# ZhendongS/Physics-Informed-Neural-Network-for-Explainable-Fault-Diagnosis-in-Fuel-Cells

Measured on AMD Instinct MI355X. Metric: pinn_train_samples_per_s, higher is better.
Workload: dtype f32 (split-operand matrix products on the 16-bit matrix cores, f32 accumulate, fp32-matmul accuracy: 2 fp16 parts / 3 MFMAs per product in forward, backward and weight gradients); 1 GPU; BASELINE configs[1]: 1000000 synthetic rows x 8 features per GPU, PINN [8,256,256,256,1] + variance head, step = train_dnn (fwd+NLL+bwd+wgrad+allreduce+Adam) + one iteration of each of the 5 physics stages; rows_per_gpu=1000000, global_rows=1000000, parallelism=dp1, precision=f32x6, backend=none (single process), world_size=1

## Files before the change

physics-informed-neural-network-for-explainable-fault-diagnosis-in-fuel-cells_amd/csrc/pinn_x6_core.h:

```cpp
#pragma once
#include <type_traits>
#include <utility>
#include "pinn_bf16_core.h"

namespace pinn {
namespace x6 {

template <int I>
using IC = std::integral_constant<int, I>;
template <typename F, int... I>
__device__ __forceinline__ void static_for_impl(F&& f, std::integer_sequence<int, I...>) {
  (f(IC<I>{}), ...);
}
template <int N, typename F>
__device__ __forceinline__ void static_for(F&& f) {
  static_for_impl(f, std::make_integer_sequence<int, N>{});
}

constexpr int kThreadsX = 512;
constexpr int kTileRowsX = 128;
constexpr int kCopyLds = 16384;
constexpr int kSlabBytes = 3 * kCopyLds;

struct Mat {
  unsigned off;
  int nrb_log;
  int kp_log = 0;
  int rows_log = -1;
};
constexpr int clog2(int v) { return v <= 1 ? 0 : 1 + clog2(v >> 1); }

__device__ __forceinline__ int swz(int row) { return (0x78 >> (2 * ((row >> 2) & 3))) & 3; }

typedef __attribute__((address_space(1))) const void* gptr_t;
typedef __attribute__((address_space(3))) void* lptr_t;

#ifdef PINN_ABL_PLAINSTORE
#define PINN_STASH_ST(p, v) (*(p) = (v))
#else
#define PINN_STASH_ST(p, v) __builtin_nontemporal_store((v), (p))
#endif
#ifdef PINN_ABL_NTRING
#define PINN_RING_AUX 2
#else
#define PINN_RING_AUX 0
#endif
#ifdef PINN_X6_STAMP
__device__ unsigned long long g_x6_stamps[8 * 8];
__device__ __forceinline__ unsigned long long stamp() {
  unsigned long long t;
  __builtin_amdgcn_sched_barrier(0);
  asm volatile("s_memtime %0\n\ts_waitcnt lgkmcnt(0)" : "=s"(t) :: "memory");
  __builtin_amdgcn_sched_barrier(0);
  return t;
}
#define PINN_STAMP(pipe, k) do { const unsigned long long t_ = stamp(); (pipe).seg[k] += t_ - (pipe).last; (pipe).last = t_; } while (0)
#else
#define PINN_STAMP(pipe, k) do { } while (0)
#endif

template <int NCOPY>
struct PipeT {
  static constexpr int kSlab = NCOPY * kCopyLds;
#ifdef PINN_X6_STAMP
  unsigned long long seg[8], last;
#endif
  __amdgpu_buffer_rsrc_t rsrc;
  unsigned copy_bytes;
  char* lds;
  int par, wave;
  int read_off;
  unsigned lane_row2, lane_kq8;

  __device__ __forceinline__ void init(const void* packed, unsigned copy_bytes_, int tid) {
    rsrc = __builtin_amdgcn_make_buffer_rsrc(const_cast<void*>(packed), 0, 0x7FFFFFFF, 0x00020000);
    copy_bytes = __builtin_amdgcn_readfirstlane(copy_bytes_);
    wave = __builtin_amdgcn_readfirstlane(tid >> 6);
    read_off = 0;
    const int lane = tid & 63;
    lane_row2 = (unsigned)(lane >> 2) << 1;
    lane_kq8 = (unsigned)(((lane & 3) ^ swz(lane >> 2)) << 4);
  }
  template <int KP_LOG, int WAVES = 8>
  __device__ __forceinline__ void piece(const Mat& m, int g, int j, int buf) {
    int p = wave + WAVES * j;
    const int n = NCOPY << m.nrb_log;
    p = p < n ? p : p - n;
    asm volatile("" : "+s"(p));
    const int rs = m.rows_log >= 0 ? m.rows_log : m.nrb_log + 4;
    const unsigned voff = (lane_row2 << 5) + lane_kq8;
    const int copy = p >> m.nrb_log, rb = p & ((1 << m.nrb_log) - 1);
    const unsigned soff = (unsigned)copy * copy_bytes + 2u * (m.off + (((unsigned)g << rs) << 5) + (unsigned)rb * 512u);
    char* dst = lds + buf * kSlab + copy * kCopyLds + rb * 1024;
#ifndef PINN_ABL_NOPIECE
    __builtin_amdgcn_raw_ptr_buffer_load_lds(rsrc, (lptr_t)dst, 16, voff, soff, 0, 0);
#endif
  }
  template <int KP_LOG>
  __device__ __forceinline__ unsigned wave_base(const Mat& m) const { return 2u * m.off + (unsigned)wave * 1024u; }
  template <int KP_LOG, int WAVES, int NRB_LOG, int J>
  __device__ __forceinline__ void piece_s(unsigned mbase, int g, int buf) {
    constexpr int q = WAVES * J, copy = q >> NRB_LOG, rb0 = q & ((1 << NRB_LOG) - 1);
    static_assert(WAVES <= (1 << NRB_LOG) && copy < NCOPY, "piece_s: shape not separable");
    mbase = __builtin_amdgcn_readfirstlane(mbase);
    asm volatile("" : "+s"(mbase));
    const unsigned voff = (lane_row2 << 5) + lane_kq8;
    const unsigned soff = mbase + (unsigned)copy * copy_bytes + ((unsigned)g << (NRB_LOG + 10)) + (unsigned)rb0 * 1024u;
    char* dst = lds + buf * kSlab + wave * 1024 + copy * kCopyLds + rb0 * 1024;
#ifndef PINN_ABL_NOPIECE
    __builtin_amdgcn_raw_ptr_buffer_load_lds(rsrc, (lptr_t)dst, 16, voff, soff, 0, 0);
#endif
  }
  template <int KP_LOG, int WAVES = 8>
  __device__ __forceinline__ void prime(const Mat& first) {
    par = 0;
#pragma unroll
    for (int j = 0; j < 16 * NCOPY / WAVES; ++j)
      if (WAVES * j < (NCOPY << first.nrb_log)) piece<KP_LOG, WAVES>(first, 0, j, 0);
// ... 298 lines not shown
          PINN_STASH_ST(sp + r * 16, v0[r]);
          PINN_STASH_ST(sp + (16 + r) * 16, v1[r]);
        }
      }
    }
  }
}

template <typename S, int P, int NG, int NTOUT, int KPM, int KPN, int NPM, int NPN, bool kHasOut, int WAVES = 8, int kStIn = 0, int kStOut = 0,
          int NRBM = -1, typename FI, typename FO>
__device__ __forceinline__ void layer_x6(f32x4 (&acc)[NTOUT], typename S::Pipe& pipe, const Mat& mine, const Mat& next, int lane, PrepT<S>& st,
                                         FI&& prep_in, FO&& prep_out, bool out_on = true) {
  constexpr int kSlots = NTOUT / 2, kPerDma = (16 * S::kCopies / WAVES + kSlots - 1) / kSlots;
  constexpr int kFirst = kHasOut ? 2 : 0, kAvail = NTOUT - kFirst;
  static_assert(kAvail >= 1, "no chunk left for the next layer's group 0");
  static_assert(NRBM < 0 || NPM == (S::kCopies << NRBM), "NRBM does not match the piece count");
#ifdef PINN_ABL_GENERIC_PIECE
  constexpr int kNrbm = -1;
#else
  constexpr int kNrbm = NRBM;
#endif
  const unsigned mine_base = kNrbm >= 0 ? pipe.template wave_base<KPM>(mine) : 0u;
  static_for<NG>([&](auto gc) {
    constexpr int g = decltype(gc)::value;
    auto dma = [&](auto slotc) {
      static_for<kPerDma>([&](auto qc) {
        constexpr int j = decltype(slotc)::value * kPerDma + decltype(qc)::value;
        if constexpr (g + 1 < NG) {
          if constexpr (WAVES * j < NPM) {
            if constexpr (kNrbm >= 0) pipe.template piece_s<KPM, WAVES, kNrbm, j>(mine_base, g + 1, pipe.par ^ 1);
            else pipe.template piece<KPM, WAVES>(mine, g + 1, j, pipe.par ^ 1);
          }
        } else {
          if constexpr (WAVES * j < NPN) pipe.template piece<KPN, WAVES>(next, 0, j, pipe.par ^ 1);
        }
      });
    };
    auto vchunk = [&](auto cc) {
      constexpr int c = decltype(cc)::value;
      static_for<7>([&](auto kc) {
        constexpr int k = decltype(kc)::value;
        if constexpr ((k < 6 && kFirst + k * kAvail / 6 == c) || (k == 6 && c == NTOUT - 1)) {
          if constexpr (g + 1 < NG) prep_in(IC<g + 1>{}, IC<k>{}, st.buf[(P + g + 1) & 1]);
          else if constexpr (kHasOut) prep_out(IC<k>{}, st.buf[(P + g + 1) & 1]);
        }
      });
    };
    slab_mfma<S, NTOUT>(acc, st.buf[(P + g) & 1], pipe.cur(), lane, vchunk, dma);
    PINN_STAMP(pipe, (NTOUT == 16 ? 0 : NTOUT == 8 ? 1 : 2));
    if constexpr (g + 1 < NG) pipe.template advance<kStIn>();
    else if constexpr (kHasOut && kStOut > 0) { if (out_on) pipe.template advance<kStOut>(); else pipe.template advance<0>(); }
    else pipe.template advance<0>();
    PINN_STAMP(pipe, 4 + (NTOUT == 16 ? 0 : NTOUT == 8 ? 1 : 2));
  });
}

template <typename S, int kThreads>
__device__ __forceinline__ void fill_small(float* small, float* w0t, const float* __restrict__ params, const ParamLayout& L) {
  const SmallLayout SL{L.H, L.nh};
  const int Hh = L.H, tid = threadIdx.x;
  constexpr int kMaxH = 256, kPer = (kMaxH + kThreads - 1) / kThreads;
  constexpr int kW0 = (8 * kMaxH + kThreads - 1) / kThreads, kMaxLayers = 8;
  float vb[kMaxLayers][kPer], vwp[kPer], vbv0[kPer], vbv1[kPer], vwv2[kPer], vw0[kW0], vbp = 0.f, vbv2 = 0.f;
#pragma unroll
  for (int l = 0; l < kMaxLayers; ++l)
#pragma unroll
    for (int k = 0; k < kPer; ++k) { const int i = tid + k * kThreads; vb[l][k] = (l < L.nh && i < Hh) ? params[L.b(l) + i] : 0.f; }
#pragma unroll
  for (int k = 0; k < kPer; ++k) {
    const int i = tid + k * kThreads;
    vwp[k] = i < Hh ? params[L.wp() + i] : 0.f;
    vbv0[k] = i < Hh / 2 ? params[L.bv0() + i] : 0.f;
    vbv1[k] = i < Hh / 4 ? params[L.bv1() + i] : 0.f;
    vwv2[k] = i < Hh / 4 ? params[L.wv2() + i] : 0.f;
  }
#pragma unroll
  for (int k = 0; k < kW0; ++k) { const int e = tid + k * kThreads; vw0[k] = e < Hh * 8 ? params[L.w0() + e] : 0.f; }
  if (tid == 0) { vbp = params[L.bp()]; vbv2 = params[L.bv2()]; }
#pragma unroll
  for (int l = 0; l < kMaxLayers; ++l)
#pragma unroll
    for (int k = 0; k < kPer; ++k) { const int i = tid + k * kThreads; if (l < L.nh && i < Hh) small[SL.b(l) + i] = l == 0 ? vb[l][k] : vb[l][k] * S::kAccScale; }
#pragma unroll
  for (int k = 0; k < kPer; ++k) {
    const int i = tid + k * kThreads;
    if (i < Hh) small[SL.wp() + i] = vwp[k];
    if (i < Hh / 2) small[SL.bv0() + i] = vbv0[k] * S::kAccScale;
    if (i < Hh / 4) { small[SL.bv1() + i] = vbv1[k] * S::kAccScale; small[SL.wv2() + i] = vwv2[k]; }
  }
#pragma unroll
  for (int k = 0; k < kW0; ++k) { const int e = tid + k * kThreads; if (e < Hh * 8) w0t[(e & 7) * kW0Stride + (e >> 3)] = vw0[k]; }
  if (tid == 0) { small[SL.bp()] = vbp; small[SL.bv2()] = vbv2; }
  __syncthreads();
}

__device__ __forceinline__ int lane_of(const RowCtx& c) { return c.lane; }

template <int H>
__device__ __forceinline__ Mat first_mat(const PackLayout& K) {
  return K.nh > 1 ? Mat{(unsigned)K.w(1), clog2(H / 16)} : Mat{(unsigned)K.wv0(), clog2(H / 32)};
}

__device__ __forceinline__ float* packed_ptr(float* base, long long t16, int F, int lane) {
  return base + t16 * F * 16 + (lane & 15) * 16 + (lane >> 4) * 4;
}

struct StashX {
  float* h; float* v1; float* v2;
  float* dh; float* dv1; float* dv2;
  long long t16_total, t16;
  __device__ __forceinline__ float* act(int layer, int H_, int lane) const {
    return tiled_ptr(h + (long long)layer * t16_total * H_ * 16, t16, H_, lane);
  }
  __device__ __forceinline__ float* dact(int layer, int H_, int lane) const {
    return tiled_ptr(dh + (long long)layer * t16_total * H_ * 16, t16, H_, lane);
  }
  __device__ __forceinline__ float* actp(int layer, int H_, int lane) const {
    return packed_ptr(h + (long long)layer * t16_total * H_ * 16, t16, H_, lane);
  }
  __device__ __forceinline__ float* dactp(int layer, int H_, int lane) const {
    return packed_ptr(dh + (long long)layer * t16_total * H_ * 16, t16, H_, lane);
  }
};

template <typename S, int H, bool kBits, bool TRAIN = false, int WAVES = 8, bool kPack = false>
__device__ __forceinline__ void forward_pass(const float* w0t, const float* smallp, const ParamLayout& L, typename S::Pipe& pipe,
                                             const DropDev& d, const RowCtx& c, const f32x4& xa, const f32x4& xb, float& u, float& z,
                                             const StashX* sx = nullptr) {
  static_assert(!kPack || (TRAIN && S::kCopies == 2), "the packed stash holds scheme X3's fragments");
  constexpr int NT = H / 16, NT2 = H / 32, NT4 = H / 64, NP = H / 32, NC = S::kCopies;
  constexpr int kSt = TRAIN ? (kPack ? 2 : 8) : 0;
  auto act_ptr = [&](int layer) -> float* { return kPack ? sx->actp(layer, H, lane_of(c)) : sx->act(layer, H, lane_of(c)); };
  auto v1_ptr = [&]() -> float* { return kPack ? packed_ptr(sx->v1, sx->t16, H / 2, lane_of(c)) : tiled_ptr(sx->v1, sx->t16, H / 2, lane_of(c)); };
  using Frag = typename S::Frag;
  const int lane = c.lane, kq = c.kq;
  const SmallLayout SL{L.H, L.nh};
  const PackLayout K{L.H, L.nh};
  constexpr int KPW = clog2(H), KPV1 = clog2((H / 2 + 63) & ~63);
  const Mat m_v0{(unsigned)K.wv0(), clog2(H / 32)}, m_v1{(unsigned)K.wv1(), clog2(H / 64)};
  const float* wp = smallp + SL.wp();
  const int ll = L.nh - 1;
  constexpr float kPre0 = kTanhPre, kPreS = kTanhPre / S::kAccScale;
  auto drop_of = [&](int layer) { LayerDrop ld = layer_drop(d, c.mode, layer); ld.scale *= S::kActScale; return ld; };
  float up = 0.0f;
  PrepT<S> st;
  f32x4 h[NT];
  layer_input_lds<NT>(h, w0t, smallp + SL.b(0), xa, xb, lane);
  {
    const LayerDrop ld0 = drop_of(0);
    float* sp = TRAIN ? act_ptr(0) : nullptr;
    static_for<7>([&](auto kc) { prep_micro<S, kBits, true, decltype(kc)::value, 0, kPack>(st, h[0], h[1], d, c, ld0, kPre0, 0, wp, up, ll == 0, st.buf[0], sp); });
  }
#pragma unroll 1
  for (int l = 1; l < L.nh; ++l) {
    f32x4 acc[NT];
    bias_blocks<NT>(acc, smallp + SL.b(l), kq);
    const LayerDrop ld_in = drop_of(l - 1), ld_out = drop_of(l);
    const float pre_in = l == 1 ? kPre0 : kPreS;
    const bool last = l == ll;
    const Mat mine{(unsigned)K.w(l), clog2(H / 16)}, next = last ? m_v0 : Mat{(unsigned)K.w(l + 1), clog2(H / 16)};
    float* sp_in = TRAIN ? act_ptr(l - 1) : nullptr;
    float* sp_out = TRAIN ? act_ptr(l) : nullptr;
    static_assert(NP % 2 == 0 && (NP / 2) % 2 == 0, "the forward layers keep the fragment buffer parity");
    layer_x6<S, 0, NP, NT, KPW, KPW, NC * H / 16, NC * H / 16, true, WAVES, kSt, kSt, clog2(H / 16)>(
        acc, pipe, mine, next, lane, st,
        [&](auto gc, auto kc, Frag& out) {
          constexpr int g = decltype(gc)::value;
          prep_micro<S, kBits, false, decltype(kc)::value, g, kPack>(st, h[2 * g], h[2 * g + 1], d, c, ld_in, pre_in, l - 1, wp, up, false, out,
                                                                    TRAIN ? sp_in + 32 * g * 16 : nullptr);
        },
        [&](auto kc, Frag& out) {
          prep_micro<S, kBits, true, decltype(kc)::value, 0, kPack>(st, acc[0], acc[1], d, c, ld_out, kPreS, l, wp, up, last, out, sp_out);
        });
#pragma unroll
    for (int t = 0; t < NT; ++t) h[t] = acc[t];
  }
  f32x4 v1[NT2];
  bias_blocks<NT2>(v1, smallp + SL.bv0(), kq);
  {
    const LayerDrop ld_in = drop_of(ll), ld_out = drop_of(L.nh);
    const float pre_in = ll == 0 ? kPre0 : kPreS;
    float* sp_in = TRAIN ? act_ptr(ll) : nullptr;
    float* sp_out = TRAIN ? v1_ptr() : nullptr;
    layer_x6<S, 0, NP, NT2, KPW, KPV1, NC * H / 32, NC * H / 64, true, WAVES, kSt, kSt, (WAVES <= H / 32 ? clog2(H / 32) : -1)>(
        v1, pipe, m_v0, m_v1, lane, st,
        [&](auto gc, auto kc, Frag& out) {
          constexpr int g = decltype(gc)::value;
          prep_micro<S, kBits, true, decltype(kc)::value, g, kPack>(st, h[2 * g], h[2 * g + 1], d, c, ld_in, pre_in, ll, wp + 32 * g, up, true, out,
                                                                   TRAIN ? sp_in + 32 * g * 16 : nullptr);
        },
        [&](auto kc, Frag& out) {
          prep_micro<S, kBits, false, decltype(kc)::value, 0, kPack>(st, v1[0], v1[1], d, c, ld_out, kPreS, L.nh, wp, up, false, out, sp_out);
        });
  }
  u = sum_kq(up) + smallp[SL.bp()];
  f32x4 v2[NT4];
  bias_blocks<NT4>(v2, smallp + SL.bv1(), kq);
  {
    const LayerDrop ld_in = drop_of(L.nh);
    float* sp_in = TRAIN ? v1_ptr() : nullptr;
    auto prep_in = [&](auto gc, auto kc, Frag& out) {
      constexpr int g = decltype(gc)::value;
      prep_micro<S, kBits, false, decltype(kc)::value, g, kPack>(st, v1[2 * g], v1[2 * g + 1], d, c, ld_in, kPreS, L.nh, wp, up, false, out,
                                                                TRAIN ? sp_in + 32 * g * 16 : nullptr);
    };
// ... 29 lines not shown
};

struct StashFrag {
  u32x4 hi, lo;
};
template <int B, int R>
__device__ __forceinline__ float unpack_act(const StashFrag& f) {
  const unsigned hw = f.hi[R], lw = f.lo[R];
  const f16x2 h = __builtin_bit_cast(f16x2, hw), l = __builtin_bit_cast(f16x2, lw);
  return (float)h[B] + (float)l[B];
}

__device__ __forceinline__ int grad_exponent(float mx, int e_if_zero) {
  int e = 0;
  (void)frexpf(mx, &e);
  return (mx > 0.0f && mx < __builtin_inff()) ? (e < -120 ? -120 : e) : e_if_zero;
}

template <typename S, int k>
__device__ __forceinline__ void bprep_micro(typename S::Frag& out, f32x4& d0, f32x4& d1, const StashRing& ring, int buf, float* dsp, float gscale,
                                            float inv_scale, float unnorm, float& mx, StashFrag& sf) {
  constexpr bool kPack = S::kCopies == 2;
  if constexpr (k == 1) {
    if constexpr (kPack) { sf.hi = ring.read_frag(buf, 0); sf.lo = ring.read_frag(buf, 1); }
  } else if constexpr (k >= 2 && k < 6) {
    constexpr int r = k - 2;
    const float h0 = kPack ? unpack_act<0, r>(sf) : ring.read(buf, 0, r), h1 = kPack ? unpack_act<1, r>(sf) : ring.read(buf, 1, r);
    const float a0 = h0 * inv_scale, a1 = h1 * inv_scale;
    const float g0 = d0[r] * (gscale * (1.0f - a0 * a0)), g1 = d1[r] * (gscale * (1.0f - a1 * a1));
    const float p0 = h0 != 0.0f ? g0 : 0.0f, p1 = h1 != 0.0f ? g1 : 0.0f;
    d0[r] = p0; d1[r] = p1;
    S::template split<r>(p0, p1, out);
  } else if constexpr (k == 6) {
    if constexpr (kPack) {
      PINN_STASH_ST(reinterpret_cast<u32x4*>(dsp), out.hi);
      PINN_STASH_ST(reinterpret_cast<u32x4*>(dsp + 256), out.lo);
#pragma unroll
      for (int r = 0; r < 4; ++r) mx = fmaxf(fmaxf(mx, fabsf(d0[r])), fabsf(d1[r]));
    } else {
#pragma unroll
      for (int r = 0; r < 4; ++r) {
        PINN_STASH_ST(dsp + r * 16, S::kActScale != 1.0f ? d0[r] * unnorm : d0[r]);
        PINN_STASH_ST(dsp + (16 + r) * 16, S::kActScale != 1.0f ? d1[r] * unnorm : d1[r]);
        if constexpr (S::kActScale != 1.0f) mx = fmaxf(fmaxf(mx, fabsf(d0[r])), fabsf(d1[r]));
      }
    }
  }
}

struct RowMeta {
  _Float16* rec;
  int E, c;
};
template <typename S, int H, int WAVES = 8>
__device__ __forceinline__ void backward_pass(const float* smallp, const ParamLayout& L, typename S::Pipe& pipe, const DropDev& d, int mode,
                                              const StashX& sx, const StashRing& ring, int lane, float du, float dz, float& amax,
                                              const RowMeta meta = RowMeta{nullptr, 4, 0}) {
  constexpr int NT = H / 16, NT2 = H / 32, NT4 = H / 64, NP = H / 32, NC = S::kCopies;
  constexpr int NG1 = (H / 4) / 32 > 0 ? (H / 4) / 32 : 1;
  constexpr int KPW = clog2(H), KPT0 = clog2((H / 2 + 63) & ~63), KPT1 = clog2((H / 4 + 63) & ~63);
  constexpr bool kPack = NC == 2;
  constexpr int kSt = kPack ? 2 : 8;
  using Frag = typename S::Frag;
  const int kq = lane >> 4;
  const SmallLayout SL{L.H, L.nh};
  const PackLayout K{L.H, L.nh};
  const int nh = L.nh;
  const int n_blocks = NP / 2 + (nh - 1) * NP;
  auto block_ptr = [&](int i) -> const float* {
    if (i < NP / 2) return sx.v1 + (sx.t16 * (H / 2) + 32 * i) * 16;
    const int j = i - NP / 2, layer = nh - 1 - j / NP, g = j % NP;
    return sx.h + ((long long)layer * sx.t16_total * H + sx.t16 * H + 32 * g) * 16;
  };
  auto fetch_block = [&](int i) {
    if (i < n_blocks) ring.fetch(block_ptr(i), i & 1);
  };
  fetch_block(0);

  float unnorm = 1.0f;
  float mx = 0.0f;
  if constexpr (S::kActScale != 1.0f) {
    const int e = grad_exponent(fmaxf(fabsf(du), fabsf(dz)), kPack ? meta.E : 4);
    const float norm = ldexpf(1.0f, 4 - e);
    unnorm = ldexpf(1.0f, e - 4);
    if constexpr (kPack) {
      if (meta.rec && lane < 16) reinterpret_cast<float*>(meta.rec)[32 + lane] = dz;
    }
    du *= norm; dz *= norm;
    if constexpr (kPack) {
      if (meta.rec && lane < 16) {
        const _Float16 dh16 = (_Float16)du;
        meta.rec[lane] = (_Float16)ldexpf(1.0f, e - meta.E + meta.c);
        meta.rec[16 + lane] = dh16;
        meta.rec[32 + lane] = (_Float16)(du - (float)dh16);
      }
    }
  }
  constexpr float kInvW = 1.0f / (S::kAccScale / S::kActScale);
  constexpr float kInvA = kPack ? 1.0f / S::kActScale : 1.0f;

  PrepT<S> st;
  StashFrag sf;
  constexpr int P1 = NG1 & 1;
  f32x4 v2[NT4];
  float* dsp2 = kPack ? packed_ptr(sx.dv2, sx.t16, H / 4, lane) : tiled_ptr(sx.dv2, sx.t16, H / 4, lane);
  {
    const float* vp = tiled_ptr(sx.v2, sx.t16, H / 4, lane);
#pragma unroll
    for (int t = 0; t < NT4; ++t) load_block(vp, t, v2[t]);
#pragma unroll
    for (int t = 0; t < NT4; ++t) {
      const f32x4 w = *reinterpret_cast<const f32x4*>(smallp + SL.wv2() + t * 16 + 4 * kq);
      f32x4 true_units;
#pragma unroll
      for (int r = 0; r < 4; ++r) {
        v2[t][r] = w[r] * dz * (1.0f - v2[t][r] * v2[t][r]);
        true_units[r] = v2[t][r] * unnorm;
        if constexpr (S::kActScale != 1.0f) mx = fmaxf(mx, fabsf(v2[t][r]));
      }
      if constexpr (!kPack) store_block(dsp2, t, true_units);
    }
    const f32x4 zero = {0.f, 0.f, 0.f, 0.f};
    const f32x4& second = NT4 >= 2 ? v2[NT4 >= 2 ? 1 : 0] : zero;
    static_for<4>([&](auto rc) { constexpr int r = decltype(rc)::value; S::template split<r>(v2[0][r], second[r], st.buf[0]); });
    if constexpr (kPack) {
      PINN_STASH_ST(reinterpret_cast<u32x4*>(dsp2), st.buf[0].hi);
      PINN_STASH_ST(reinterpret_cast<u32x4*>(dsp2 + 256), st.buf[0].lo);
    }
  }
  const Mat m_t1{(unsigned)K.wv1t(), clog2(H / 32)}, m_t0{(unsigned)K.wv0t(), clog2(H / 16)};
  const Mat m_again{m_t1.off, m_t1.nrb_log, KPT1};
  auto dv1_ptr = [&]() -> float* { return kPack ? packed_ptr(sx.dv1, sx.t16, H / 2, lane) : tiled_ptr(sx.dv1, sx.t16, H / 2, lane); };
  auto dact_ptr = [&](int layer) -> float* { return kPack ? sx.dactp(layer, H, lane) : sx.dact(layer, H, lane); };

  f32x4 dpv1[NT2];
  zero_blocks<NT2>(dpv1);
  {
    const LayerDrop ldv = layer_drop(d, mode, nh);
    const float gscale = ldv.scale * kInvW, inv_scale = kInvA / ldv.scale;
    float* dsp = dv1_ptr();
    layer_x6<S, 0, NG1, NT2, KPT1, KPT0, NC * H / 32, NC * H / 16, true, WAVES, (kPack ? 2 : 0), kSt, (WAVES <= H / 32 ? clog2(H / 32) : -1)>(
        dpv1, pipe, m_t1, m_t0, lane, st,
        [&](auto gc, auto kc, Frag& out) {
          constexpr int g = decltype(gc)::value, k = decltype(kc)::value;
          if constexpr (k >= 2 && k < 6 && 2 * g + 1 < NT4) S::template split<k - 2>(v2[2 * g][k - 2], v2[2 * g + 1][k - 2], out);
          if constexpr (kPack && k == 6 && 2 * g + 1 < NT4) {
            PINN_STASH_ST(reinterpret_cast<u32x4*>(dsp2 + 512 * g), out.hi);
            PINN_STASH_ST(reinterpret_cast<u32x4*>(dsp2 + 512 * g + 256), out.lo);
          }
        },
        [&](auto kc, Frag& out) {
          constexpr int k = decltype(kc)::value;
          if constexpr (k == 0) {
            asm volatile("s_waitcnt vmcnt(0)" ::: "memory");
            fetch_block(1);
          }
          bprep_micro<S, k>(out, dpv1[0], dpv1[1], ring, 0, dsp, gscale, inv_scale, unnorm, mx, sf);
        });
  }

  f32x4 dh[NT];
#pragma unroll
  for (int t = 0; t < NT; ++t) {
    const f32x4 w = *reinterpret_cast<const f32x4*>(smallp + SL.wp() + t * 16 + 4 * kq);
    dh[t] = w * (du * (S::kAccScale / S::kActScale));
  }
  {
    const LayerDrop ldv = layer_drop(d, mode, nh), ldh = layer_drop(d, mode, nh - 1);
    const float gscale = ldv.scale * kInvW, inv_scale = kInvA / ldv.scale, gscale_o = ldh.scale * kInvW, inv_scale_o = kInvA / ldh.scale;
    float* dsp = dv1_ptr();
    float* dsp_o = dact_ptr(nh - 1);
    const Mat next = nh > 1 ? Mat{(unsigned)K.wt(nh - 1), clog2(H / 16), KPW} : m_again;
    layer_x6<S, P1, NP / 2, NT, KPT0, -1, NC * H / 16, NC * H / 16, true, WAVES, kSt, kSt, clog2(H / 16)>(
        dh, pipe, m_t0, next, lane, st,
        [&](auto gc, auto kc, Frag& out) {
          constexpr int g = decltype(gc)::value, k = decltype(kc)::value;
          if constexpr (k == 0) fetch_block(g + 1);
          bprep_micro<S, k>(out, dpv1[2 * g], dpv1[2 * g + 1], ring, g & 1, dsp + 32 * g * 16, gscale, inv_scale, unnorm, mx, sf);
        },
        [&](auto kc, Frag& out) {
          constexpr int k = decltype(kc)::value;
          if (nh > 1) {
            if constexpr (k == 0) fetch_block(NP / 2 + 1);
            bprep_micro<S, k>(out, dh[0], dh[1], ring, (NP / 2) & 1, dsp_o, gscale_o, inv_scale_o, unnorm, mx, sf);
          }
        },
        nh > 1);
  }

#pragma unroll 1
  for (int l = nh - 1; l >= 1; --l) {
    f32x4 acc[NT];
    zero_blocks<NT>(acc);
    const LayerDrop ld_in = layer_drop(d, mode, l), ld_out = layer_drop(d, mode, l - 1);
    const float gscale = ld_in.scale * kInvW, inv_scale = kInvA / ld_in.scale, gscale_o = ld_out.scale * kInvW, inv_scale_o = kInvA / ld_out.scale;
    float* dsp = dact_ptr(l);
    float* dsp_o = dact_ptr(l - 1);
    const int base = NP / 2 + (nh - 1 - l) * NP;
    const Mat mine{(unsigned)K.wt(l), clog2(H / 16)}, next = l > 1 ? Mat{(unsigned)K.wt(l - 1), clog2(H / 16), KPW} : m_again;
    layer_x6<S, P1, NP, NT, KPW, -1, NC * H / 16, NC * H / 16, true, WAVES, kSt, kSt, clog2(H / 16)>(
        acc, pipe, mine, next, lane, st,
        [&](auto gc, auto kc, Frag& out) {
          constexpr int g = decltype(gc)::value, k = decltype(kc)::value;
          if constexpr (k == 0) fetch_block(base + g + 1);
          bprep_micro<S, k>(out, dh[2 * g], dh[2 * g + 1], ring, (base + g) & 1, dsp + 32 * g * 16, gscale, inv_scale, unnorm, mx, sf);
        },
        [&](auto kc, Frag& out) {
          constexpr int k = decltype(kc)::value;
          if (l > 1) {
            if constexpr (k == 0) fetch_block(base + NP + 1);
            bprep_micro<S, k>(out, acc[0], acc[1], ring, (base + NP) & 1, dsp_o, gscale_o, inv_scale_o, unnorm, mx, sf);
          }
        },
        l > 1);
#pragma unroll
    for (int t = 0; t < NT; ++t) dh[t] = acc[t];
  }

  {
    const LayerDrop ld0 = layer_drop(d, mode, 0);
    const float gscale = ld0.scale * kInvW * (kPack ? 1.0f : unnorm), inv_scale = kInvA / ld0.scale;
    auto one = [&](float h, float dv) -> float {
      const float a0 = h * inv_scale;
      const float g0 = dv * (gscale * (1.0f - a0 * a0));
      return h != 0.0f ? g0 : 0.0f;
    };
    if constexpr (kPack) {
      const float* hp = sx.actp(0, H, lane);
      float* dsp = sx.dactp(0, H, lane);
      StashFrag fr[NP];
// ... 40 lines not shown
```

physics-informed-neural-network-for-explainable-fault-diagnosis-in-fuel-cells_amd/csrc/pinn_x6_train.hip:

```cpp
#include <cstdlib>
#include "pinn_x6_core.h"

namespace pinn {
namespace x6 {

struct TrainArgsX {
  const float* params;
  const float* x;
  const float* y;
  long long n_rows, n_global;
  int H, nh;
  DropDev drop;
  TrainBuffers b;
};

template <int H, bool kBits, int WAVES, bool kPack>
__global__ __launch_bounds__(WAVES * 64, WAVES / 4) void train_fwd_x3_kernel(TrainArgsX a, const __bf16* packed) {
  using S = X3;
  constexpr int kThreadsX = WAVES * 64, kTileRowsX = WAVES * 16;
  constexpr int kSmallBytes = kMaxSmall * 4, kW0Bytes = 8 * kW0Stride * 4, kRedBytes = 8 * kLossTerms * 8;
  constexpr int kSlabAt = (kSmallBytes + kW0Bytes + kRedBytes + 1023) & ~1023;
  __shared__ __attribute__((aligned(1024))) char smem[kSlabAt + 2 * S::Pipe::kSlab];
  float* small = reinterpret_cast<float*>(smem);
  float* w0t = reinterpret_cast<float*>(smem + kSmallBytes);
  double (*red)[kLossTerms] = reinterpret_cast<double (*)[kLossTerms]>(smem + kSmallBytes + kW0Bytes);
  char* lds_w = smem + kSlabAt;
  ParamLayout L{a.H, a.nh};
  PackLayout K{a.H, a.nh};
  fill_small<S, kThreadsX>(small, w0t, a.params, L);
  S::Pipe pipe;
  pipe.lds = lds_w;
  pipe.init(packed + 3 * K.total(), (unsigned)(K.total() * 2), threadIdx.x);
  pipe.template prime<clog2(H), WAVES>(first_mat<H>(K));

  const int lane = threadIdx.x & 63, wave = pipe.wave, kq = lane >> 4;
  const float inv_n = (float)(1.0 / (double)a.n_global);
  LossSums sums;
  float gmax = 0.f;
  if (blockIdx.x == 0 && threadIdx.x == 0) *a.b.amax = 0u;

  const long long n_tiles = (a.n_rows + 127) / 128 * (128 / kTileRowsX);
  const unsigned pass0 = train_pass(a.drop);
  if (blockIdx.x == 0 && threadIdx.x == 0) a.b.amax[2] = pass0;
  for (long long tile = blockIdx.x; tile < n_tiles; tile += gridDim.x) {
    const long long t16 = tile * WAVES + wave;
    const long long lrow = t16 * 16 + (lane & 15);
    const bool valid = lrow < a.n_rows;
    const long long srow = valid ? lrow : a.n_rows - 1;
    const f32x4 xa = reinterpret_cast<const f32x4*>(a.x)[srow * 2];
    const f32x4 xb = reinterpret_cast<const f32x4*>(a.x)[srow * 2 + 1];
    const float yv = a.y[srow];
    const RowCtx c{lane, kq, a.drop.row_offset + lrow, srow, a.n_rows, pass0, a.drop.mode};
    const StashX sx{(float*)a.b.stash_h, (float*)a.b.stash_v1, (float*)a.b.stash_v2, (float*)a.b.dpre_h, (float*)a.b.dpre_v1, (float*)a.b.dpre_v2,
                    a.b.t16, t16};

    if constexpr (kPack) {
      Frag2 fx;
      static_for<4>([&](auto rc) {
        constexpr int r = decltype(rc)::value;
        const float v = kq == 0 ? xa[r] : (kq == 1 ? xb[r] : 0.0f);
        S::template split<r>(v * 0.0625f, 0.0f, fx);
      });
      float* xp = packed_ptr((float*)a.b.stash_x, t16, 32, lane);
      PINN_STASH_ST(reinterpret_cast<u32x4*>(xp), fx.hi);
      PINN_STASH_ST(reinterpret_cast<u32x4*>(xp + 256), fx.lo);
    }
    float u, z;
    forward_pass<S, H, kBits, true, WAVES, kPack>(w0t, small, L, pipe, a.drop, c, xa, xb, u, z, &sx);

    float du, dz;
    loss_row(u, z, yv, inv_n, valid, kq == 0, du, dz, sums);
    if (lane < 16) { a.b.du[t16 * 16 + lane] = du; a.b.dz[t16 * 16 + lane] = dz; }
    gmax = fmaxf(gmax, fmaxf(fabsf(du), fabsf(dz)));
  }
  if constexpr (kPack) wave_max_to(a.b.emax, gmax, lane == 0);

  store_loss_partials<WAVES>(sums, red, a.b.loss_part, lane, wave);
}

template <typename S, int H, int WAVES>
__global__ __launch_bounds__(WAVES * 64, WAVES / 4) void train_bwd_kernel(TrainArgsX a, const __bf16* packed) {
  constexpr int kThreadsX = WAVES * 64, kTileRowsX = WAVES * 16;
  constexpr int kSmallBytes = kMaxSmall * 4, kW0Bytes = 8 * kW0Stride * 4, kRingBytes = 8 * 2 * 2048;
  constexpr int kSlabAt = (kSmallBytes + kW0Bytes + kRingBytes + 1023) & ~1023;
  __shared__ __attribute__((aligned(1024))) char smem[kSlabAt + 2 * S::Pipe::kSlab];
  float* small = reinterpret_cast<float*>(smem);
  float* w0t = reinterpret_cast<float*>(smem + kSmallBytes);
  char* ring_lds = smem + kSmallBytes + kW0Bytes;
  char* lds_w = smem + kSlabAt;
  ParamLayout L{a.H, a.nh};
  PackLayout K{a.H, a.nh};
  fill_small<X6, kThreadsX>(small, w0t, a.params, L);
  typename S::Pipe pipe;
  pipe.lds = lds_w;
  pipe.init(packed + (S::kCopies == 2 ? 3 * K.total() : 0), (unsigned)(K.total() * 2), threadIdx.x);
  constexpr int KPT1 = clog2((H / 4 + 63) & ~63);
  pipe.template prime<KPT1, WAVES>(Mat{(unsigned)K.wv1t(), clog2(H / 32)});

  const int lane = threadIdx.x & 63, wave = pipe.wave;
  const StashRing ring{ring_lds + wave * 4096, lane};
  const long long n_tiles = (a.n_rows + 127) / 128 * (128 / kTileRowsX);
  float amax = 0.0f;
  int E = 4;
  if constexpr (S::kCopies == 2) E = grad_exponent(__builtin_bit_cast(float, __builtin_amdgcn_readfirstlane(*a.b.emax)), 4);
  for (long long tile = blockIdx.x; tile < n_tiles; tile += gridDim.x) {
    const long long t16 = tile * WAVES + wave;
    const StashX sx{(float*)a.b.stash_h, (float*)a.b.stash_v1, (float*)a.b.stash_v2, (float*)a.b.dpre_h, (float*)a.b.dpre_v1, (float*)a.b.dpre_v2,
                    a.b.t16, t16};
    const float du = a.b.du[t16 * 16 + (lane & 15)], dz = a.b.dz[t16 * 16 + (lane & 15)];
    const RowMeta meta{S::kCopies == 2 ? (_Float16*)a.b.rowmeta + t16 * 128 : nullptr, E, a.b.qboost};
    backward_pass<S, H, WAVES>(small, L, pipe, a.drop, a.drop.mode, sx, ring, lane, du, dz, amax, meta);
  }
  if constexpr (S::kActScale != 1.0f) wave_max_to(a.b.amax, amax, lane == 0);
}

#ifdef PINN_ABL_Q_NTSTORE
#define PINN_Q_ST(p, v) __builtin_nontemporal_store((v), (p))
#else
#define PINN_Q_ST(p, v) (*(p) = (v))
#endif
struct Xch {
  char* base;
  int off;
  __device__ __forceinline__ u32x4 read(int g, int part) const { return *reinterpret_cast<const u32x4*>(base + g * 2048 + part * 1024 + off); }
  __device__ __forceinline__ void write(int g, const Frag2& f) const {
    *reinterpret_cast<u32x4*>(base + g * 2048 + off) = f.hi;
    *reinterpret_cast<u32x4*>(base + g * 2048 + 1024 + off) = f.lo;
  }
};
__device__ __forceinline__ void lds_barrier() {
  asm volatile("s_waitcnt lgkmcnt(0)" ::: "memory");
  __builtin_amdgcn_s_barrier();
  asm volatile("" ::: "memory");
}
template <bool kDot>
__device__ __forceinline__ void prep_group(Frag2& out, const f32x4& v0, const f32x4& v1, const DropDev& d, const RowCtx& c, const LayerDrop ld,
                                           float pre, int layer, int fp, const float* wp32, float& up) {
  unsigned keep = 0u;
  if (c.mode == PINN_DROP_BITS) {
    const unsigned word = d.bits[((long long)c.pass * c.n_rows + c.lrow) * d.words + layer * d.nb + fp];
    const unsigned lo = (word >> (4 * c.kq)) & 0xFu, hi = (word >> (16 + 4 * c.kq)) & 0xFu;
    keep = ld.thr == 0 ? 0xFFu : (lo | (hi << 4));
  } else {
    PrepBase s;
    s.w0 = (unsigned)c.grow; s.w1 = (unsigned)((unsigned long long)c.grow >> 32);
    s.w2 = ((unsigned)layer << 16) | ((unsigned)fp << 2) | (unsigned)c.kq; s.w3 = d.stream + c.pass;
    philox_rounds5<0>(s, d.seed_lo, d.seed_hi);
    philox_rounds5<5>(s, d.seed_lo, d.seed_hi);
    static_for<4>([&](auto rc) {
      constexpr int r = decltype(rc)::value;
      keep |= (keep_draw<0, r>(s, ld.thr) ? 1u : 0u) << r;
      keep |= (keep_draw<1, r>(s, ld.thr) ? 1u : 0u) << (4 + r);
    });
  }
  const float m2s = -2.0f * ld.scale;
  static_for<4>([&](auto rc) {
    constexpr int r = decltype(rc)::value;
    float a0 = fmaf(m2s, __builtin_amdgcn_rcpf(__builtin_amdgcn_exp2f(v0[r] * pre) + 1.0f), ld.scale);
    float a1 = fmaf(m2s, __builtin_amdgcn_rcpf(__builtin_amdgcn_exp2f(v1[r] * pre) + 1.0f), ld.scale);
    a0 = a0 == 0.0f ? 0x1p-24f : a0;
    a1 = a1 == 0.0f ? 0x1p-24f : a1;
    const float hs0 = ((keep >> r) & 1u) ? a0 : 0.0f, hs1 = ((keep >> (4 + r)) & 1u) ? a1 : 0.0f;
    X3::split<r>(hs0, hs1, out);
    if constexpr (kDot) {
      const float h0 = hs0 * (1.0f / X3::kActScale), h1 = hs1 * (1.0f / X3::kActScale);
// ... 304 lines not shown
int train_chain_x6_partials(const pinn_net_t* net, long long n_rows) { return x6::plan_chain(net, n_rows).grid_fwd; }

int launch_train_chain_x6(const pinn_net_t* net, const float* d_params, const float* d_x, const float* d_y, long long n_rows,
                          long long n_global, const DropDev& drop, const TrainBuffers& b, unsigned which, void* stream) {
  using namespace x6;
  hipStream_t st = (hipStream_t)stream;
  const bool fast_bwd = net->precision == PINN_PREC_F32X6;
  const bool run_fwd = which & 1u, fwd_only = !(which & 2u);
  launch_pack_x6(net, d_params, st, fast_bwd && run_fwd ? b.emax : nullptr);
  TrainArgsX a{};
  a.params = d_params; a.x = d_x; a.y = d_y; a.n_rows = n_rows; a.n_global = n_global; a.H = net->hidden; a.nh = net->n_hidden;
  a.drop = drop; a.b = b;
  const ChainPlan c = plan_chain(net, n_rows);
  const bool small_n = c.small_n;
  const int grid = c.grid;
  const __bf16* packed = (const __bf16*)net->d_packed;
  const bool bits = drop.mode == PINN_DROP_BITS;
  if (c.quarters) {
    if (run_fwd) hipLaunchKernelGGL((train_fwd_small_kernel<256>), dim3(c.grid_fwd), dim3(kSmallThreads), 0, st, a, packed);
    if (!fwd_only) {
      if (!run_fwd) { hipError_t em = hipMemsetAsync(b.amax, 0, sizeof(unsigned), st); if (em != hipSuccess) return (int)em; }
      hipLaunchKernelGGL((train_bwd_kernel<X3, 256, 4>), dim3(grid), dim3(256), 0, st, a, packed);
    }
    hipError_t eq = hipGetLastError();
    return eq == hipSuccess ? PINN_OK : (int)eq;
  }
  if (fast_bwd && !fwd_only && !run_fwd) {
    hipError_t em = hipMemsetAsync(b.amax, 0, sizeof(unsigned), st);
    if (em != hipSuccess) return (int)em;
  }
#define PINN_LAUNCH_T(HH, BB)                                                                                                   \
  do {                                                                                                                          \
    if (small_n) {                                                                                                              \
      if (run_fwd && fast_bwd) hipLaunchKernelGGL((train_fwd_x3_kernel<HH, BB, 4, true>), dim3(grid), dim3(256), 0, st, a, packed);   \
      else if (run_fwd) hipLaunchKernelGGL((train_fwd_x3_kernel<HH, BB, 4, false>), dim3(grid), dim3(256), 0, st, a, packed);   \
      if (!fwd_only && fast_bwd) hipLaunchKernelGGL((train_bwd_kernel<X3, HH, 4>), dim3(grid), dim3(256), 0, st, a, packed);    \
      else if (!fwd_only) hipLaunchKernelGGL((train_bwd_kernel<X6, HH, 4>), dim3(grid), dim3(256), 0, st, a, packed);           \
    } else {                                                                                                                    \
      if (run_fwd && fast_bwd) hipLaunchKernelGGL((train_fwd_x3_kernel<HH, BB, 8, true>), dim3(grid), dim3(512), 0, st, a, packed);   \
      else if (run_fwd) hipLaunchKernelGGL((train_fwd_x3_kernel<HH, BB, 8, false>), dim3(grid), dim3(512), 0, st, a, packed);   \
      if (!fwd_only && fast_bwd) hipLaunchKernelGGL((train_bwd_kernel<X3, HH, 8>), dim3(grid), dim3(512), 0, st, a, packed);    \
      else if (!fwd_only) hipLaunchKernelGGL((train_bwd_kernel<X6, HH, 8>), dim3(grid), dim3(512), 0, st, a, packed);           \
    }                                                                                                                           \
  } while (0)
  if (net->hidden == 256) { if (bits) PINN_LAUNCH_T(256, true); else PINN_LAUNCH_T(256, false); }
  else { if (bits) PINN_LAUNCH_T(128, true); else PINN_LAUNCH_T(128, false); }
#undef PINN_LAUNCH_T
  hipError_t e = hipGetLastError();
  return e == hipSuccess ? PINN_OK : (int)e;
}

}

#ifdef PINN_Q_STAMP
extern "C" int pinn_q_debug_read(unsigned long long* host) {
  return (int)hipMemcpyFromSymbol(host, HIP_SYMBOL(pinn::x6::g_q_stamps), sizeof(unsigned long long) * 8 * 16);
}
#endif
```

Baseline: 227.6 million samples/s.

## Prefetch next tile's inputs into LDS across the tile seam in fwd and bwd kernels

In the forward kernel, each wave's x/y rows for the next tile are fetched into a double-buffered LDS stage with global_load_lds, issued after the first layer prep. In the backward kernel, the next tile's du/dz, v2 stash and first v1 ring block are fetched during the current tile. The first fetches are issued before fill_small and weight priming so they overlap. The aim is to hide global-load latency at tile boundaries, at the cost of extra LDS and a removed vmcnt wait that could create ordering hazards. Optional seam timing stamps are added behind a macro.

```diff
diff --git a/physics-informed-neural-network-for-explainable-fault-diagnosis-in-fuel-cells_amd/csrc/pinn_x6_core.h b/physics-informed-neural-network-for-explainable-fault-diagnosis-in-fuel-cells_amd/csrc/pinn_x6_core.h
--- a/physics-informed-neural-network-for-explainable-fault-diagnosis-in-fuel-cells_amd/csrc/pinn_x6_core.h
+++ b/physics-informed-neural-network-for-explainable-fault-diagnosis-in-fuel-cells_amd/csrc/pinn_x6_core.h
@@ -58,12 +58,32 @@
 #else
 #define PINN_STAMP(pipe, k) do { } while (0)
 #endif
+#ifdef PINN_SEAM_STAMP
+__device__ __forceinline__ unsigned long long seam_now() {
+  unsigned long long t;
+  __builtin_amdgcn_sched_barrier(0);
+  asm volatile("s_memtime %0\n\ts_waitcnt lgkmcnt(0)" : "=s"(t) :: "memory");
+  __builtin_amdgcn_sched_barrier(0);
+  return t;
+}
+#define PINN_SEAM_BEGIN(pipe) do { (pipe).seam_t0 = seam_now(); (pipe).seam_first = 0; } while (0)
+#define PINN_SEAM_MARK(pipe) do { const unsigned long long t_ = seam_now(); if ((pipe).seam_first == 0) (pipe).seam_first = t_; (pipe).seam_last = t_; } while (0)
+#define PINN_SEAM_END(pipe) do { const unsigned long long t_ = seam_now(); (pipe).seam_acc[0] += (pipe).seam_first - (pipe).seam_t0; \
+    (pipe).seam_acc[1] += (pipe).seam_last - (pipe).seam_first; (pipe).seam_acc[2] += t_ - (pipe).seam_last; (pipe).seam_acc[3] += 1; } while (0)
+#else
+#define PINN_SEAM_BEGIN(pipe) do { } while (0)
+#define PINN_SEAM_MARK(pipe) do { } while (0)
+#define PINN_SEAM_END(pipe) do { } while (0)
+#endif
 
 template <int NCOPY>
 struct PipeT {
   static constexpr int kSlab = NCOPY * kCopyLds;
 #ifdef PINN_X6_STAMP
   unsigned long long seg[8], last;
+#endif
+#ifdef PINN_SEAM_STAMP
+  unsigned long long seam_t0, seam_first, seam_last, seam_acc[4];
 #endif
   __amdgpu_buffer_rsrc_t rsrc;
   unsigned copy_bytes;
@@ -468,6 +488,7 @@
     else if constexpr (kHasOut && kStOut > 0) { if (out_on) pipe.template advance<kStOut>(); else pipe.template advance<0>(); }
     else pipe.template advance<0>();
     PINN_STAMP(pipe, 4 + (NTOUT == 16 ? 0 : NTOUT == 8 ? 1 : 2));
+    PINN_SEAM_MARK(pipe);
   });
 }
 
@@ -539,10 +560,33 @@
   }
 };
 
-template <typename S, int H, bool kBits, bool TRAIN = false, int WAVES = 8, bool kPack = false>
+struct RowStage {
+  static constexpr int kBytes = 1024 + 256;
+  char* lds;
+  __device__ __forceinline__ void fetch(const float* x, const float* y, long long t16, long long n_rows, int lane, int buf) const {
+    asm volatile("" : "+v"(lane));
+    const long long rx = t16 * 16 + ((lane & 31) >> 1), ry = t16 * 16 + (lane & 15);
+    const char* xs = reinterpret_cast<const char*>(x) + (rx < n_rows ? rx : n_rows - 1) * 32 + (lane & 1) * 16;
+    const float* ys = y + (ry < n_rows ? ry : n_rows - 1);
+    __builtin_amdgcn_global_load_lds((gptr_t)xs, (lptr_t)(lds + buf * kBytes), 16, 0, 0);
+    __builtin_amdgcn_global_load_lds((gptr_t)ys, (lptr_t)(lds + buf * kBytes + 1024), 4, 0, 0);
+  }
+  __device__ __forceinline__ void read(int buf, int lane, f32x4& xa, f32x4& xb, float& yv) const {
+    asm volatile("" : "+v"(lane));
+    const unsigned ax = (unsigned)(unsigned long long)(lptr_t)(lds + buf * kBytes) + (unsigned)(lane & 15) * 32u;
+    const unsigned ay = (unsigned)(unsigned long long)(lptr_t)(lds + buf * kBytes + 1024) + (unsigned)(lane & 15) * 4u;
+    asm volatile("ds_read_b128 %0, %3\n\tds_read_b128 %1, %3 offset:16\n\tds_read_b32 %2, %4\n\ts_waitcnt lgkmcnt(0)"
+                 : "=&v"(xa), "=&v"(xb), "=&v"(yv) : "v"(ax), "v"(ay) : "memory");
+  }
+};
+
+struct NoHook {
+  __device__ __forceinline__ void operator()() const {}
+};
+template <typename S, int H, bool kBits, bool TRAIN = false, int WAVES = 8, bool kPack = false, typename Hook = NoHook>
 __device__ __forceinline__ void forward_pass(const float* w0t, const float* smallp, const ParamLayout& L, typename S::Pipe& pipe,
                                              const DropDev& d, const RowCtx& c, const f32x4& xa, const f32x4& xb, float& u, float& z,
-                                             const StashX* sx = nullptr) {
+                                             const StashX* sx = nullptr, const Hook& first_step = Hook()) {
   static_assert(!kPack || (TRAIN && S::kCopies == 2), "the packed stash holds scheme X3's fragments");
   constexpr int NT = H / 16, NT2 = H / 32, NT4 = H / 64, NP = H / 32, NC = S::kCopies;
   constexpr int kSt = TRAIN ? (kPack ? 2 : 8) : 0;
@@ -567,6 +611,11 @@
     float* sp = TRAIN ? act_ptr(0) : nullptr;
     static_for<7>([&](auto kc) { prep_micro<S, kBits, true, decltype(kc)::value, 0, kPack>(st, h[0], h[1], d, c, ld0, kPre0, 0, wp, up, ll == 0, st.buf[0], sp); });
   }
+  if constexpr (!std::is_same_v<Hook, NoHook>) {
+    __builtin_amdgcn_sched_barrier(0);
+    first_step();
+    __builtin_amdgcn_sched_barrier(0);
+  }
 #pragma unroll 1
   for (int l = 1; l < L.nh; ++l) {
     f32x4 acc[NT];
@@ -702,10 +751,36 @@
   _Float16* rec;
   int E, c;
 };
+template <int H, bool kV2>
+struct TileSeam {
+  static constexpr int kV2Bytes = kV2 ? (H / 4) * 16 * 4 : 0, kBytes = 256 + kV2Bytes;
+  char* lds;
+  const float* du;
+  const float* dz;
+  const float* v2;
+  long long t16_next;
+  __device__ __forceinline__ void fetch(long long t16, int lane) const {
+    const float* g = ((lane & 16) ? dz : du) + t16 * 16 + (lane & 15);
+    __builtin_amdgcn_global_load_lds((gptr_t)g, (lptr_t)lds, 4, 0, 0);
+    if constexpr (kV2) {
+      const char* v = reinterpret_cast<const char*>(v2 + t16 * (H / 4) * 16) + lane * 16;
+#pragma unroll
+      for (int j = 0; j < kV2Bytes / 1024; ++j)
+        __builtin_amdgcn_global_load_lds((gptr_t)(v + j * 1024), (lptr_t)(lds + 256 + j * 1024), 16, 0, 0);
+    }
+  }
+  __device__ __forceinline__ float du_of(int lane) const { return reinterpret_cast<const float*>(lds)[lane & 15]; }
+  __device__ __forceinline__ float dz_of(int lane) const { return reinterpret_cast<const float*>(lds)[16 + (lane & 15)]; }
+  __device__ __forceinline__ void v2_block(int t, int lane, f32x4& v) const {
+    const float* p = reinterpret_cast<const float*>(lds + 256) + (4 * (lane >> 4)) * 16 + (lane & 15);
+#pragma unroll
+    for (int r = 0; r < 4; ++r) v[r] = p[(t * 16 + r) * 16];
+  }
+};
 template <typename S, int H, int WAVES = 8>
 __device__ __forceinline__ void backward_pass(const float* smallp, const ParamLayout& L, typename S::Pipe& pipe, const DropDev& d, int mode,
                                               const StashX& sx, const StashRing& ring, int lane, float du, float dz, float& amax,
-                                              const RowMeta meta = RowMeta{nullptr, 4, 0}) {
+                                              const RowMeta meta, const TileSeam<H, S::kCopies == 2>& seam) {
   constexpr int NT = H / 16, NT2 = H / 32, NT4 = H / 64, NP = H / 32, NC = S::kCopies;
   constexpr int NG1 = (H / 4) / 32 > 0 ? (H / 4) / 32 : 1;
   constexpr int KPW = clog2(H), KPT0 = clog2((H / 2 + 63) & ~63), KPT1 = clog2((H / 4 + 63) & ~63);
@@ -722,10 +797,11 @@
     const int j = i - NP / 2, layer = nh - 1 - j / NP, g = j % NP;
     return sx.h + ((long long)layer * sx.t16_total * H + sx.t16 * H + 32 * g) * 16;
   };
+  static_assert((NP / 2) % 2 == 0 && NP % 2 == 0, "n_blocks is even: the next tile's block 0 goes to ring buffer 0");
   auto fetch_block = [&](int i) {
     if (i < n_blocks) ring.fetch(block_ptr(i), i & 1);
+    else if (i == n_blocks && seam.t16_next >= 0) ring.fetch(sx.v1 + seam.t16_next * (H / 2) * 16, 0);
   };
-  fetch_block(0);
 
   float unnorm = 1.0f;
   float mx = 0.0f;
@@ -755,9 +831,14 @@
   f32x4 v2[NT4];
   float* dsp2 = kPack ? packed_ptr(sx.dv2, sx.t16, H / 4, lane) : tiled_ptr(sx.dv2, sx.t16, H / 4, lane);
   {
-    const float* vp = tiled_ptr(sx.v2, sx.t16, H / 4, lane);
-#pragma unroll
-    for (int t = 0; t < NT4; ++t) load_block(vp, t, v2[t]);
+    if constexpr (kPack) {
+#pragma unroll
+      for (int t = 0; t < NT4; ++t) seam.v2_block(t, lane, v2[t]);
+    } else {
+      const float* vp = tiled_ptr(sx.v2, sx.t16, H / 4, lane);
+#pragma unroll
+      for (int t = 0; t < NT4; ++t) load_block(vp, t, v2[t]);
+    }
 #pragma unroll
     for (int t = 0; t < NT4; ++t) {
       const f32x4 w = *reinterpret_cast<const f32x4*>(smallp + SL.wv2() + t * 16 + 4 * kq);
@@ -801,10 +882,7 @@
         },
         [&](auto kc, Frag& out) {
           constexpr int k = decltype(kc)::value;
-          if constexpr (k == 0) {
-            asm volatile("s_waitcnt vmcnt(0)" ::: "memory");
-            fetch_block(1);
-          }
+          if constexpr (k == 0) fetch_block(1);
           bprep_micro<S, k>(out, dpv1[0], dpv1[1], ring, 0, dsp, gscale, inv_scale, unnorm, mx, sf);
         });
   }
@@ -825,7 +903,10 @@
         dh, pipe, m_t0, next, lane, st,
         [&](auto gc, auto kc, Frag& out) {
           constexpr int g = decltype(gc)::value, k = decltype(kc)::value;
-          if constexpr (k == 0) fetch_block(g + 1);
+          if constexpr (k == 0) {
+            fetch_block(g + 1);
+            if constexpr (g == 1) { if (seam.t16_next >= 0) seam.fetch(seam.t16_next, lane); }
+          }
           bprep_micro<S, k>(out, dpv1[2 * g], dpv1[2 * g + 1], ring, g & 1, dsp + 32 * g * 16, gscale, inv_scale, unnorm, mx, sf);
         },
         [&](auto kc, Frag& out) {
diff --git a/physics-informed-neural-network-for-explainable-fault-diagnosis-in-fuel-cells_amd/csrc/pinn_x6_train.hip b/physics-informed-neural-network-for-explainable-fault-diagnosis-in-fuel-cells_amd/csrc/pinn_x6_train.hip
--- a/physics-informed-neural-network-for-explainable-fault-diagnosis-in-fuel-cells_amd/csrc/pinn_x6_train.hip
+++ b/physics-informed-neural-network-for-explainable-fault-diagnosis-in-fuel-cells_amd/csrc/pinn_x6_train.hip
@@ -14,12 +14,23 @@
   TrainBuffers b;
 };
 
+#ifdef PINN_SEAM_STAMP
+__device__ unsigned long long g_seam_stamps[2 * 8 * 4];
+#define PINN_SEAM_INIT(pipe) do { for (int k_ = 0; k_ < 4; ++k_) (pipe).seam_acc[k_] = 0; } while (0)
+#define PINN_SEAM_OUT(pipe, kernel) do { if (blockIdx.x == 0 && (threadIdx.x & 63) == 0) for (int k_ = 0; k_ < 4; ++k_) \
+    g_seam_stamps[((kernel) * 8 + (pipe).wave) * 4 + k_] = (pipe).seam_acc[k_]; } while (0)
+#else
+#define PINN_SEAM_INIT(pipe) do { } while (0)
+#define PINN_SEAM_OUT(pipe, kernel) do { } while (0)
+#endif
+
 template <int H, bool kBits, int WAVES, bool kPack>
 __global__ __launch_bounds__(WAVES * 64, WAVES / 4) void train_fwd_x3_kernel(TrainArgsX a, const __bf16* packed) {
   using S = X3;
   constexpr int kThreadsX = WAVES * 64, kTileRowsX = WAVES * 16;
   constexpr int kSmallBytes = kMaxSmall * 4, kW0Bytes = 8 * kW0Stride * 4, kRedBytes = 8 * kLossTerms * 8;
-  constexpr int kSlabAt = (kSmallBytes + kW0Bytes + kRedBytes + 1023) & ~1023;
+  constexpr int kStageAt = (kSmallBytes + kW0Bytes + kRedBytes + 15) & ~15, kStageBytes = WAVES * 2 * RowStage::kBytes;
+  constexpr int kSlabAt = (kStageAt + kStageBytes + 1023) & ~1023;
   __shared__ __attribute__((aligned(1024))) char smem[kSlabAt + 2 * S::Pipe::kSlab];
   float* small = reinterpret_cast<float*>(smem);
   float* w0t = reinterpret_cast<float*>(smem + kSmallBytes);
@@ -27,29 +38,39 @@
   char* lds_w = smem + kSlabAt;
   ParamLayout L{a.H, a.nh};
   PackLayout K{a.H, a.nh};
-  fill_small<S, kThreadsX>(small, w0t, a.params, L);
   S::Pipe pipe;
   pipe.lds = lds_w;
   pipe.init(packed + 3 * K.total(), (unsigned)(K.total() * 2), threadIdx.x);
+  const int lane = threadIdx.x & 63, wave = pipe.wave, kq = lane >> 4;
+  const long long n_tiles = (a.n_rows + 127) / 128 * (128 / kTileRowsX);
+  const RowStage rows{smem + kStageAt + wave * 2 * RowStage::kBytes};
+  if ((long long)blockIdx.x < n_tiles) rows.fetch(a.x, a.y, (long long)blockIdx.x * WAVES + wave, a.n_rows, lane, 0);
+  fill_small<S, kThreadsX>(small, w0t, a.params, L);
   pipe.template prime<clog2(H), WAVES>(first_mat<H>(K));
-
-  const int lane = threadIdx.x & 63, wave = pipe.wave, kq = lane >> 4;
+  asm volatile("s_waitcnt vmcnt(0)" ::: "memory");
+
   const float inv_n = (float)(1.0 / (double)a.n_global);
   LossSums sums;
   float gmax = 0.f;
   if (blockIdx.x == 0 && threadIdx.x == 0) *a.b.amax = 0u;
 
-  const long long n_tiles = (a.n_rows + 127) / 128 * (128 / kTileRowsX);
   const unsigned pass0 = train_pass(a.drop);
   if (blockIdx.x == 0 && threadIdx.x == 0) a.b.amax[2] = pass0;
-  for (long long tile = blockIdx.x; tile < n_tiles; tile += gridDim.x) {
+  PINN_SEAM_INIT(pipe);
+  int rbuf = 0;
+  for (long long tile = blockIdx.x; tile < n_tiles; tile += gridDim.x, rbuf ^= 1) {
+    PINN_SEAM_BEGIN(pipe);
     const long long t16 = tile * WAVES + wave;
     const long long lrow = t16 * 16 + (lane & 15);
     const bool valid = lrow < a.n_rows;
     const long long srow = valid ? lrow : a.n_rows - 1;
-    const f32x4 xa = reinterpret_cast<const f32x4*>(a.x)[srow * 2];
-    const f32x4 xb = reinterpret_cast<const f32x4*>(a.x)[srow * 2 + 1];
-    const float yv = a.y[srow];
+    f32x4 xa, xb;
+    float yv;
+    rows.read(rbuf, lane, xa, xb, yv);
+    const long long tile_next = tile + gridDim.x;
+    auto prefetch = [&]() {
+      if (tile_next < n_tiles) rows.fetch(a.x, a.y, tile_next * WAVES + wave, a.n_rows, lane, rbuf ^ 1);
+    };
     const RowCtx c{lane, kq, a.drop.row_offset + lrow, srow, a.n_rows, pass0, a.drop.mode};
     const StashX sx{(float*)a.b.stash_h, (float*)a.b.stash_v1, (float*)a.b.stash_v2, (float*)a.b.dpre_h, (float*)a.b.dpre_v1, (float*)a.b.dpre_v2,
                     a.b.t16, t16};
@@ -66,13 +87,15 @@
       PINN_STASH_ST(reinterpret_cast<u32x4*>(xp + 256), fx.lo);
     }
     float u, z;
-    forward_pass<S, H, kBits, true, WAVES, kPack>(w0t, small, L, pipe, a.drop, c, xa, xb, u, z, &sx);
+    forward_pass<S, H, kBits, true, WAVES, kPack>(w0t, small, L, pipe, a.drop, c, xa, xb, u, z, &sx, prefetch);
 
     float du, dz;
     loss_row(u, z, yv, inv_n, valid, kq == 0, du, dz, sums);
     if (lane < 16) { a.b.du[t16 * 16 + lane] = du; a.b.dz[t16 * 16 + lane] = dz; }
     gmax = fmaxf(gmax, fmaxf(fabsf(du), fabsf(dz)));
-  }
+    PINN_SEAM_END(pipe);
+  }
+  PINN_SEAM_OUT(pipe, 0);
   if constexpr (kPack) wave_max_to(a.b.emax, gmax, lane == 0);
 
   store_loss_partials<WAVES>(sums, red, a.b.loss_part, lane, wave);
@@ -82,7 +105,9 @@
 __global__ __launch_bounds__(WAVES * 64, WAVES / 4) void train_bwd_kernel(TrainArgsX a, const __bf16* packed) {
   constexpr int kThreadsX = WAVES * 64, kTileRowsX = WAVES * 16;
   constexpr int kSmallBytes = kMaxSmall * 4, kW0Bytes = 8 * kW0Stride * 4, kRingBytes = 8 * 2 * 2048;
-  constexpr int kSlabAt = (kSmallBytes + kW0Bytes + kRingBytes + 1023) & ~1023;
+  using Seam = TileSeam<H, S::kCopies == 2>;
+  constexpr int kSeamAt = (kSmallBytes + kW0Bytes + kRingBytes + 15) & ~15;
+  constexpr int kSlabAt = (kSeamAt + WAVES * Seam::kBytes + 1023) & ~1023;
   __shared__ __attribute__((aligned(1024))) char smem[kSlabAt + 2 * S::Pipe::kSlab];
   float* small = reinterpret_cast<float*>(smem);
   float* w0t = reinterpret_cast<float*>(smem + kSmallBytes);
@@ -90,27 +115,38 @@
   char* lds_w = smem + kSlabAt;
   ParamLayout L{a.H, a.nh};
   PackLayout K{a.H, a.nh};
-  fill_small<X6, kThreadsX>(small, w0t, a.params, L);
   typename S::Pipe pipe;
   pipe.lds = lds_w;
   pipe.init(packed + (S::kCopies == 2 ? 3 * K.total() : 0), (unsigned)(K.total() * 2), threadIdx.x);
-  constexpr int KPT1 = clog2((H / 4 + 63) & ~63);
-  pipe.template prime<KPT1, WAVES>(Mat{(unsigned)K.wv1t(), clog2(H / 32)});
-
   const int lane = threadIdx.x & 63, wave = pipe.wave;
   const StashRing ring{ring_lds + wave * 4096, lane};
   const long long n_tiles = (a.n_rows + 127) / 128 * (128 / kTileRowsX);
+  Seam seam{smem + kSeamAt + wave * Seam::kBytes, a.b.du, a.b.dz, (const float*)a.b.stash_v2, -1};
+  if ((long long)blockIdx.x < n_tiles) {
+    const long long t16 = (long long)blockIdx.x * WAVES + wave;
+    seam.fetch(t16, lane);
+    ring.fetch((const float*)a.b.stash_v1 + t16 * (H / 2) * 16, 0);
+  }
+  fill_small<X6, kThreadsX>(small, w0t, a.params, L);
+  constexpr int KPT1 = clog2((H / 4 + 63) & ~63);
+  pipe.template prime<KPT1, WAVES>(Mat{(unsigned)K.wv1t(), clog2(H / 32)});
+  asm volatile("s_waitcnt vmcnt(0)" ::: "memory");
   float amax = 0.0f;
   int E = 4;
   if constexpr (S::kCopies == 2) E = grad_exponent(__builtin_bit_cast(float, __builtin_amdgcn_readfirstlane(*a.b.emax)), 4);
+  PINN_SEAM_INIT(pipe);
   for (long long tile = blockIdx.x; tile < n_tiles; tile += gridDim.x) {
+    PINN_SEAM_BEGIN(pipe);
     const long long t16 = tile * WAVES + wave;
     const StashX sx{(float*)a.b.stash_h, (float*)a.b.stash_v1, (float*)a.b.stash_v2, (float*)a.b.dpre_h, (float*)a.b.dpre_v1, (float*)a.b.dpre_v2,
                     a.b.t16, t16};
-    const float du = a.b.du[t16 * 16 + (lane & 15)], dz = a.b.dz[t16 * 16 + (lane & 15)];
+    const float du = seam.du_of(lane), dz = seam.dz_of(lane);
+    seam.t16_next = tile + gridDim.x < n_tiles ? (tile + gridDim.x) * WAVES + wave : -1;
     const RowMeta meta{S::kCopies == 2 ? (_Float16*)a.b.rowmeta + t16 * 128 : nullptr, E, a.b.qboost};
-    backward_pass<S, H, WAVES>(small, L, pipe, a.drop, a.drop.mode, sx, ring, lane, du, dz, amax, meta);
-  }
+    backward_pass<S, H, WAVES>(small, L, pipe, a.drop, a.drop.mode, sx, ring, lane, du, dz, amax, meta, seam);
+    PINN_SEAM_END(pipe);
+  }
+  PINN_SEAM_OUT(pipe, 1);
   if constexpr (S::kActScale != 1.0f) wave_max_to(a.b.amax, amax, lane == 0);
 }
 
@@ -521,6 +557,11 @@
 
 }
 
+#ifdef PINN_SEAM_STAMP
+extern "C" int pinn_seam_debug_read(unsigned long long* host) {
+  return (int)hipMemcpyFromSymbol(host, HIP_SYMBOL(pinn::x6::g_seam_stamps), sizeof(unsigned long long) * 2 * 8 * 4);
+}
+#endif
 #ifdef PINN_Q_STAMP
 extern "C" int pinn_q_debug_read(unsigned long long* host) {
   return (int)hipMemcpyFromSymbol(host, HIP_SYMBOL(pinn::x6::g_q_stamps), sizeof(unsigned long long) * 8 * 16);
```

Result: no change. 228.9 million samples/s, median of 6 (+0.6%).
